# wangyunpeng139/3_ORB_SLAM3_SelfNote

Hardware: AMD Instinct MI355X
Metric: frames/sec ORB extract+match, 752x480 (higher is better)
Workload: dtype u8; 1 GPU; BASELINE configs[2]: extract + SearchByProjection match, 1000x1000 candidates, synthetic frame stream; image=752x480, nfeatures=1000, nlevels=8, batch=256, distinct_frames_per_gpu=2048, streams=4

## Files before the change

### 3_orb_slam3_selfnote_amd/csrc/orb_match_kernels.h

```cpp
#pragma once
#include <hip/hip_runtime.h>
#include <stdint.h>
#include "orb_mfma_util.h"

#define MATCH_NT 256

struct MatchProblemSet {
  const float *kp;
  const uint8_t *desc;
  const float *u_right;
  int frame_stride;
  const int32_t *frame_n; int frame_n_stride; int frame_n_const;
  float min_x, min_y, inv_w, inv_h;
  const uint8_t *qdesc;
  const float *qu, *qv, *qr, *qur;
  const int32_t *qminl, *qmaxl;
  const uint8_t *qflags;
  int query_stride;
  const int32_t *query_n; int query_n_stride; int query_n_const;
  float nnratio; int th_dist; int use_second;
  int32_t *slot; uint8_t *slot_obs; int32_t *match_of_query; int32_t *best_dist; int32_t *nmatches;
  int nleft; const uint8_t *qside; const int32_t *partner; int couple; uint8_t *qany; int serial;
  const int32_t *nleft_dev; int nleft_stride;
  float inv_sigma2[16];
// ... 676 lines not shown
    K l[REFRESH_K];
#pragma unroll
    for (int j = 0; j < REFRESH_K; j++) l[j] = KT::NONE;
    const int minlE = w.checkLevels ? w.minl : -1000, maxlE = w.checkLevels && w.maxl >= 0 ? w.maxl : 1000;
    struct Probe { float x, y, ur; uint32_t bits; int c, pos; };
    auto probe = [&](int pos, bool valid) {
      Probe k;
      k.c = valid ? (int)sPerm[pos] : -1;
      k.pos = valid ? pos : 0;
      const int c = valid ? k.c : 0;
      const bool cl = sOwner[valid ? c : n] == 0u;
      if (LDSCAND) {
        const CandMeta cmeta = cMeta[k.pos];
        k.x = cmeta.x; k.y = cmeta.y; k.ur = cmeta.ur;
        k.bits = cl ? (cmeta.bits & ~(1u << 24)) : cmeta.bits;
      } else {
        k.x = kp[(size_t)c * 7]; k.y = kp[(size_t)c * 7 + 1];
        k.bits = cand_bits(k.x, k.y, __float_as_int(kp[(size_t)c * 7 + 5]), cl, M);
        k.ur = M.u_right ? M.u_right[fo + c] : -1.f;
      }
      return k;
    };
    auto passes = [&](const Probe &k) {
      const int gx = (k.bits >> 8) & 0xff, gy = (k.bits >> 16) & 0xff, oct = k.bits & 0xff;
      int viol = (gx - w.cx0) | (w.cx1 - gx) | (gy - w.cy0) | (w.cy1 - gy) | (oct - minlE) | (maxlE - oct) | k.c;
      viol |= ((k.c >= nleft) == sideR) ? 0 : -1;
      viol |= ~(int)(k.bits << 7);
      const int fpass = __float_as_int(fabsf(k.x - w.u) - w.r) & __float_as_int(fabsf(k.y - w.v) - w.r);
      bool ok = (fpass & ~viol) < 0;
      if (w.stereo) ok = ok && !(k.ur > 0.f && fabsf(w.ur - k.ur) > w.r);
      return ok;
    };
    auto score = [&](const Probe &k) {
      uint32_t d[8];
      if (LDSCAND) {
        const uint4 a = cDesc[2 * k.pos], b = cDesc[2 * k.pos + 1];
        d[0] = a.x; d[1] = a.y; d[2] = a.z; d[3] = a.w; d[4] = b.x; d[5] = b.y; d[6] = b.z; d[7] = b.w;
      } else {
#pragma unroll
        for (int t = 0; t < 8; t++) d[t] = desc[(size_t)k.c * 8 + t];
      }
      int dist = 0;
#pragma unroll
      for (int t = 0; t < 8; t++) dist += __popc(d[t] ^ q8[t]);
      K t = KT::make(dist, cell_of(k.bits), k.c);
      if (t < l[REFRESH_K - 1]) {
#pragma unroll
        for (int j = 0; j < REFRESH_K; j++) {
          const K lo = t < l[j] ? t : l[j];
          const K hi = t < l[j] ? l[j] : t;
          l[j] = lo;
          t = hi;
        }
      }
    };
    const int end = w.live ? sCol[w.cx1 + 1] : 0;
    for (int pos = (w.live ? sCol[w.cx0] : 0) + lane + 128 * part; pos < end; pos += 128 * nparts) {
      const Probe k0 = probe(pos, true);
      const Probe k1 = probe(pos + 64, pos + 64 < end);
      const bool ok0 = passes(k0), ok1 = passes(k1);
      if (ok0) score(k0);
      if (ok1) score(k1);
    }
    K out[REFRESH_K];
#pragma unroll
    for (int j = 0; j < REFRESH_K; j++) {
      out[j] = wave_min_key(l[0]);
      if (l[0] == out[j] && out[j] != KT::NONE) {
#pragma unroll
        for (int t = 0; t + 1 < REFRESH_K; t++) l[t] = l[t + 1];
        l[REFRESH_K - 1] = KT::NONE;
      }
    }
    if (lane == 0) {
#pragma unroll
      for (int j = 0; j < REFRESH_K; j++) sPart[rq][part][j] = out[j];
    }
    (void)target;
  };
  __shared__ int sVoteR;
  constexpr bool WIDE_OK = sizeof(K) == 4;
  constexpr int WN = 64 * NW_;
  constexpr int TKW_WORDS = FUSED && MATCH_TOPK * WN < 3072 ? 3072 : MATCH_TOPK * WN;
  __shared__ __align__(16) K sTkW[WIDE_OK ? TKW_WORDS : 1];
  __shared__ int sRmin[4], sChg[4], sTake, sNm;
  bool wide = false;
  if (FUSED && fusedPair) wide = false;
  else if (WIDE_OK && !M.serial && !M.partner && M.couple == 0 && !M.qside && rforce != SCAN_DENSE) {
    wide = pair_walks<WN>(M, p, n, nq, rforce, &sVoteR);
  }
  if (wide) {
    if (tid == 0) { for (int i = 0; i < 4; i++) { sRmin[i] = 0x7fffffff; sChg[i] = 0; } sTake = 0; sNm = 0; }
    __syncthreads();
    int nmatches = 0;
#ifdef WIDE_STAMPS
    long long ws_build = 0, ws_round = 0, ws_refresh = 0, ws_nround = 0, ws_nrefresh = 0, ws_ncut = 0, ws_t = __builtin_readcyclecounter();
    const long long ws_begin = ws_t;
#define WSTMP(acc) do { const long long t_ = __builtin_readcyclecounter(); acc += t_ - ws_t; ws_t = t_; } while (0)
#else
#define WSTMP(acc) do {} while (0)
#endif
    for (int base = 0; base < nq; base += WN) {
      const int q = base + tid;
      const int cnt = min(WN, nq - base);
      const uint32_t myfl = q < nq ? (M.qflags ? M.qflags[qo + q] : 3u) : 0u;
      const bool ob = (myfl >> 1) & 1u;
      uint32_t qpar[6] = {0, 0, 0, 0, 0, 0}, qd[8] = {0, 0, 0, 0, 0, 0, 0, 0};
#pragma unroll
      for (int j = 0; j < MATCH_TOPK; j++) sTkW[WN * j + tid] = q < nq ? topk[(qo + q) * MATCH_TOPK + j] : KT::NONE;
      if (q < nq) {
        qpar[0] = __float_as_uint(M.qu[qo + q]); qpar[1] = __float_as_uint(M.qv[qo + q]); qpar[2] = __float_as_uint(M.qr[qo + q]);
        qpar[3] = __float_as_uint(M.qur ? M.qur[qo + q] : 0.f);
        qpar[4] = (uint32_t)M.qminl[qo + q]; qpar[5] = (uint32_t)M.qmaxl[qo + q];
        const uint4 *qp = reinterpret_cast<const uint4 *>(M.qdesc + (qo + q) * 32);
        const uint4 a = qp[0], b = qp[1];
        qd[0] = a.x; qd[1] = a.y; qd[2] = a.z; qd[3] = a.w; qd[4] = b.x; qd[5] = b.y; qd[6] = b.z; qd[7] = b.w;
      }
      int eidx[MATCH_TOPK];
      uint32_t vm, oct4;
      int capm1 = MATCH_TOPK - 1, lbDist;
      bool truncated;
      auto load_list = [&]() {
        vm = 0; oct4 = 0;
#pragma unroll
        for (int j = 0; j < MATCH_TOPK; j++) {
          const K t = sTkW[WN * j + tid];
          eidx[j] = n;
          if (t != KT::NONE) {
            const int idx = KT::idx(t);
            eidx[j] = idx;
            vm |= 1u << j;
            oct4 |= (uint32_t)(octave_of(idx) & 0xf) << (4 * j);
          }
        }
        const K last = sTkW[WN * capm1 + tid];
        truncated = last != KT::NONE;
        lbDist = KT::dist(last);
        if (!(myfl & 1u)) { vm = 0; truncated = false; }
      };
      load_list();
      auto refresh = [&](bool want) {
        bool todo = want;
        WSTMP(ws_round);
        for (;;) {
          __syncthreads();
          int slot = -1;
          if (todo) slot = atomicAdd(&sTake, 1);
          const bool take = todo && slot < NW_;
          if (take) {
            uint32_t *R = sReq[slot];
            R[0] = (uint32_t)tid; R[1] = myfl;
#pragma unroll
            for (int t = 0; t < 6; t++) R[2 + t] = qpar[t];
#pragma unroll
            for (int t = 0; t < 8; t++) R[8 + t] = qd[t];
          }
          __syncthreads();
          const int asked = sTake;
          if (asked == 0) break;
          const int m = min(NW_, asked);
          {
            const int np = shares_of(m), mp = NW_ / np, rq = wid & (mp - 1);
            if (rq < m) serve(rq, wid / mp, np);
          }
          __syncthreads();
          if (tid == 0) sTake = 0;
          if (take) {
            static_assert(REFRESH_K == 4, "the merge network below is written for 4 keys");
            auto cx = [](K &lo, K &hi) { const K l = lo < hi ? lo : hi, h = lo < hi ? hi : lo; lo = l; hi = h; };
            const int np = shares_of(m);
            K a[REFRESH_K];
#pragma unroll
            for (int j = 0; j < REFRESH_K; j++) a[j] = sPart[slot][0][j];
            for (int sh = 1; sh < np; sh++) {
#pragma unroll
              for (int j = 0; j < REFRESH_K; j++) {
                const K y = sPart[slot][sh][REFRESH_K - 1 - j];
                a[j] = a[j] < y ? a[j] : y;
              }
              cx(a[0], a[2]); cx(a[1], a[3]);
              cx(a[0], a[1]); cx(a[2], a[3]);
            }
#pragma unroll
            for (int j = 0; j < MATCH_TOPK; j++) sTkW[WN * j + tid] = j < REFRESH_K ? a[j] : KT::NONE;
            todo = false;
            capm1 = REFRESH_K - 1;
            load_list();
          }
#ifdef WIDE_STAMPS
          ws_nrefresh++;
#endif
        }
        WSTMP(ws_refresh);
      };
      uint32_t D = 0;
      int my_bd = 256, res_idx = -1, res_bd = 256;
      int s = 0, par = 0;
      bool first_round = true;
      WSTMP(ws_build);
      while (s < cnt) {
#ifdef WIDE_STAMPS
        ws_ncut++;
#endif
        int r;
        for (;;) {
          const bool pend = tid >= s && tid < cnt;
          const bool post = pend && (D >> 31) && ob;
          const int bidx = (int)(D & 0xfffffu);
          if (post) __hip_atomic_fetch_min(&sOwner[bidx], (uint32_t)(tid + 1), __ATOMIC_RELAXED, __HIP_MEMORY_SCOPE_WORKGROUP);
          __syncthreads();
          uint32_t cm = 0;
#pragma unroll
          for (int j = 0; j < MATCH_TOPK; j++) cm |= (sOwner[eidx[j]] <= (uint32_t)tid ? 1u : 0u) << j;
          const uint32_t mine = sOwner[post ? bidx : n];
          __syncthreads();
          if (post && mine != 0u) sOwner[bidx] = RESOLVE_FREE;
          const uint32_t nD = pend ? decide<KT, WN>(M, sTkW + tid, vm, cm, oct4, truncated, lbDist, &my_bd) : D;
          const bool changed = nD != D;
          D = nD;
          const bool flagged = pend && ((D >> 30) & 1u);
          const int cur = par & 3;
          par++;
#ifdef WIDE_STAMPS
          ws_nround++;
#endif
          if (tid == 0) { sRmin[(cur + 2) & 3] = 0x7fffffff; sChg[(cur + 2) & 3] = 0; }
          if (flagged) atomicMin(&sRmin[cur], tid);
          __syncthreads();
          r = min(sRmin[cur], cnt);
          if (first_round) {
            first_round = false;
            if (r < cnt) {
              refresh(flagged);
              continue;
            }
          }
          if (changed && tid <= r) sChg[cur] = 1;
          __syncthreads();
          if (sChg[cur] == 0) break;
        }
        {
          const bool inpre = tid >= s && tid < r;
          const bool acc = inpre && (D >> 31);
          const int bidx = (int)(D & 0xfffffu);
          nmatches += __popcll(__ballot(acc));
          if (acc) {
            const int32_t sv = (int32_t)(((uint32_t)q << 1) | (ob ? 1u : 0u));
            if (ob) sOwner[bidx] = 0u;
            __hip_atomic_fetch_max(&sSlot[bidx], sv, __ATOMIC_RELAXED, __HIP_MEMORY_SCOPE_WORKGROUP);
          }
          if (inpre) { res_idx = acc ? bidx : -1; res_bd = my_bd <= M.th_dist ? my_bd : 256; }
        }
        s = r;
        if (r < cnt) refresh(tid >= r && tid < cnt && ((D >> 30) & 1u));
        else __syncthreads();
      }
      if (q < nq) {
        if (M.match_of_query) M.match_of_query[qo + q] = res_idx;
        if (M.best_dist) M.best_dist[qo + q] = res_bd;
      }
    }
    WSTMP(ws_round);
#ifdef WIDE_STAMPS
    if (tid == 0 && M.dbg) { long long *d = M.dbg + 16 * (size_t)p; d[0] = ws_build; d[1] = ws_round; d[2] = ws_refresh; d[3] = ws_nround; d[4] = ws_nrefresh; d[5] = ws_ncut; d[6] = ws_t - ws_begin; d[7] = nq; }
#endif
    if (lane == 0 && nmatches) atomicAdd(&sNm, nmatches);
    __syncthreads();
    if (tid == 0 && M.nmatches) M.nmatches[p] = sNm;
    for (int i = tid; i < n; i += 64 * NW_) {
      const int32_t v = sSlot[i];
      if (v >= 0) { slot[i] = v >> 1; slot_obs[i] = (uint8_t)(v & 1); }
    }
    return;
  }
  constexpr int CMP_CAP = 2048 / NW_;
  static_assert(!FUSED || (64 * 8 + 64 * NW_ * REFRESH_K + NW_ * CMP_CAP / 2 + NW_ * MF_TILE) * 4 <= TKW_WORDS * (int)sizeof(K), "work areas exceed the list array");
  uint32_t *sReqD = reinterpret_cast<uint32_t *>(sTkW);
  uint32_t *sPartF = sReqD + 64 * 8;
  uint16_t *sCmpF = reinterpret_cast<uint16_t *>(sPartF + 64 * NW_ * REFRESH_K);
  uint32_t *sSeedF = reinterpret_cast<uint32_t *>(sCmpF + NW_ * CMP_CAP);
  auto serve_mfma = [&](int m) __attribute__((always_inline)) {
    if constexpr (FUSED) {
      const int col = lane & 31, h = lane >> 5;
      const int nin = sCol[64];
      const int lo = (int)(((long long)nin * wid) / NW_), hi = (int)(((long long)nin * (wid + 1)) / NW_);
      uint16_t *cmp = sCmpF + wid * CMP_CAP;
      int kw = 0;
      for (int b0 = lo; b0 < hi; b0 += 64) {
        const int pos = b0 + lane;
        bool keep = false;
        if (pos < hi) keep = !(sRank[pos] & MF_REC_HELD) && sOwner[sPerm[pos]] != 0u;
        const unsigned long long mk = __ballot(keep);
        if (keep) cmp[kw + __popcll(mk & ((1ull << lane) - 1ull))] = (uint16_t)pos;
        kw += __popcll(mk);
      }
      const bool two = m > 32;
      uint32_t q0[4], q1[4];
      {
        const uint4 *r0 = reinterpret_cast<const uint4 *>(sReqD + col * 8), *r1 = reinterpret_cast<const uint4 *>(sReqD + (32 + col) * 8);
        const uint4 a0 = r0[0], b0 = r0[1], a1 = r1[0], b1 = r1[1];
        const uint32_t d0[8] = {a0.x, a0.y, a0.z, a0.w, b0.x, b0.y, b0.z, b0.w}, d1[8] = {a1.x, a1.y, a1.z, a1.w, b1.x, b1.y, b1.z, b1.w};
#pragma unroll
        for (int s = 0; s < 4; s++) {
          q0[s] = ((d0[2 * s] >> (16 * h)) & 0xffffu) | ((d0[2 * s + 1] >> (16 * h)) << 16);
          q1[s] = ((d1[2 * s] >> (16 * h)) & 0xffffu) | ((d1[2 * s + 1] >> (16 * h)) << 16);
        }
      }
      auto bq = [](const uint32_t *q, int s) { return mf_expand16((q[s >> 1] >> (16 * (s & 1))) & 0xffffu, MF_LUT_QUERY); };
      MfList<REFRESH_K> L0, L1;
      L0.init(); L1.init();
      uint32_t *seedw = sSeedF + wid * MF_TILE;
      int npos = 0;
      uint4 na = make_uint4(0u, 0u, 0u, 0u), nb = na;
      if (kw > 0) {
        npos = col < kw ? (int)cmp[col] : 0;
        na = cDesc[2 * npos]; nb = cDesc[2 * npos + 1];
      }
      for (int t0 = 0; t0 < kw; t0 += MF_TILE) {
        const bool have = t0 + col < kw;
#pragma unroll
        for (int s = 0; s < 4; s++) asm("" : "+v"(q0[s]), "+v"(q1[s]));
        const int pos = npos;
        const uint4 da = na, db = nb;
        if (t0 + MF_TILE < kw) {
          const int e2 = t0 + MF_TILE + col;
          npos = e2 < kw ? (int)cmp[e2] : 0;
          na = cDesc[2 * npos]; nb = cDesc[2 * npos + 1];
        }
        if (h == 0) seedw[col] = have ? sRank[pos] : MF_REC_UNUSABLE;
        const uint32_t dd[8] = {da.x, da.y, da.z, da.w, db.x, db.y, db.z, db.w};
        mf_v4i A[8];
#pragma unroll
        for (int s = 0; s < 8; s++) A[s] = mf_expand16((dd[s] >> (16 * h)) & 0xffffu, MF_LUT_CAND);
        mf_v16i c;
#pragma unroll
        for (int g = 0; g < 4; g++) {
          const mf_v4i v4 = *reinterpret_cast<const mf_v4i *>(&seedw[8 * g + 4 * h]);
          c[4 * g] = v4[0]; c[4 * g + 1] = v4[1]; c[4 * g + 2] = v4[2]; c[4 * g + 3] = v4[3];
        }
        mf_v16i acc0 = c;
#pragma unroll
        for (int s = 0; s < 8; s++) acc0 = __builtin_amdgcn_mfma_i32_32x32x32_i8(A[s], bq(q0, s), acc0, 0, 0, 0);
        L0.take(acc0);
        if (two) {
          mf_v16i acc1 = c;
#pragma unroll
          for (int s = 0; s < 8; s++) acc1 = __builtin_amdgcn_mfma_i32_32x32x32_i8(A[s], bq(q1, s), acc1, 0, 0, 0);
          L1.take(acc1);
        }
      }
      static_assert(REFRESH_K == 4, "the merge network below is written for 4 keys");
      uint32_t mg[REFRESH_K];
#pragma unroll
      for (int j = 0; j < REFRESH_K; j++) {
        const uint32_t send = h ? L0.top[REFRESH_K - 1 - j] : L1.top[REFRESH_K - 1 - j];
        const uint32_t other = (uint32_t)__shfl_xor((int)send, 32, 64);
        mg[j] = min(h ? L1.top[j] : L0.top[j], other);
      }
      auto cxu = [](uint32_t &a, uint32_t &b) { const uint32_t l = min(a, b), g2 = max(a, b); a = l; b = g2; };
      cxu(mg[0], mg[2]); cxu(mg[1], mg[3]);
      cxu(mg[0], mg[1]); cxu(mg[2], mg[3]);
      const int req = h * 32 + col;
      if (req < m) *reinterpret_cast<uint4 *>(sPartF + ((size_t)req * NW_ + wid) * REFRESH_K) = make_uint4(mg[0], mg[1], mg[2], mg[3]);
    }
  };
  auto fold_mfma = [&](int rank, K *colp ) {
    if constexpr (FUSED) {
      auto cxu = [](uint32_t &a, uint32_t &b) { const uint32_t l = min(a, b), g2 = max(a, b); a = l; b = g2; };
      const uint4 *sh = reinterpret_cast<const uint4 *>(sPartF + (size_t)rank * NW_ * REFRESH_K);
      uint4 v = sh[0];
      uint32_t a[REFRESH_K] = {v.x, v.y, v.z, v.w};
#pragma unroll
      for (int w2 = 1; w2 < NW_; w2++) {
        v = sh[w2];
        a[0] = min(a[0], v.w); a[1] = min(a[1], v.z); a[2] = min(a[2], v.y); a[3] = min(a[3], v.x);
        cxu(a[0], a[2]); cxu(a[1], a[3]);
        cxu(a[0], a[1]); cxu(a[2], a[3]);
      }
#pragma unroll
      for (int j = 0; j < MATCH_TOPK; j++) {
        K o = KT::NONE;
        if (j < REFRESH_K && a[j] < MF_KEY_LIMIT) o = (K)(((a[j] >> 11) << 23) | (uint32_t)sPerm[a[j] & 0x7ffu]);
        colp[64 * j] = o;
      }
    }
  };
#ifdef RESOLVE_STAMPS
  long long t_round = 0, t_refresh = 0, n_refresh = 0, n_batch = 0, t_chunk = 0, n_round = 0, t_sub[6] = {0, 0, 0, 0, 0, 0}, sub_m = 0;
  long long t0 = __builtin_readcyclecounter();
#endif
  if (wid != 0) {
    for (;;) {
      __syncthreads();
      const int m = sCmd;
      if (m < 0) break;
      if (FUSED && fusedPair) serve_mfma(m);
      else {
        const int np = shares_of(m), mp = NW_ / np, rq = wid & (mp - 1);
        if (rq < m) serve(rq, wid / mp, np);
      }
      __syncthreads();
    }
  } else {
    int nmatches = 0;
    for (int base = 0; base < nq; base += 64) {
#ifdef RESOLVE_STAMPS
      long long tc0 = __builtin_readcyclecounter();
#endif
      const int q = base + lane;
      const int cnt = min(64, nq - base);
      uint32_t myfl = q < nq ? (M.qflags ? M.qflags[qo + q] : 3u) : 0u;
      if (M.qside && q < nq && M.qside[qo + q]) myfl |= 0x100u;
      if (M.couple == 2 && (q & 1) && q < nq && !M.qany[qo + q - 1]) myfl &= ~1u;
      const bool ob = (myfl >> 1) & 1u;
      uint32_t qpar[6] = {0, 0, 0, 0, 0, 0}, qd[8] = {0, 0, 0, 0, 0, 0, 0, 0};
#pragma unroll
      for (int j = 0; j < MATCH_TOPK; j++) sTk[64 * j + lane] = (q < nq && !(FUSED && fusedPair)) ? topk[(qo + q) * MATCH_TOPK + j] : KT::NONE;
      if (q < nq) {
        qpar[0] = __float_as_uint(M.qu[qo + q]); qpar[1] = __float_as_uint(M.qv[qo + q]); qpar[2] = __float_as_uint(M.qr[qo + q]);
        qpar[3] = __float_as_uint(M.qur ? M.qur[qo + q] : 0.f);
        qpar[4] = (uint32_t)M.qminl[qo + q]; qpar[5] = (uint32_t)M.qmaxl[qo + q];
        const uint4 *qp = reinterpret_cast<const uint4 *>(M.qdesc + (qo + q) * 32);
        const uint4 a = qp[0], b = qp[1];
        qd[0] = a.x; qd[1] = a.y; qd[2] = a.z; qd[3] = a.w; qd[4] = b.x; qd[5] = b.y; qd[6] = b.z; qd[7] = b.w;
        if (FUSED && fusedPair && !load_query(M, qo, q).live) myfl &= ~1u;
      }
      int eidx[MATCH_TOPK];
      uint32_t vm, oct4;
      int capm1 = MATCH_TOPK - 1, lbDist;
      bool truncated;
      auto load_list = [&]() {
        vm = 0; oct4 = 0;
#pragma unroll
        for (int j = 0; j < MATCH_TOPK; j++) {
          const K t = sTk[64 * j + lane];
          eidx[j] = n;
          if (t != KT::NONE) {
            const int idx = KT::idx(t);
            eidx[j] = idx;
            vm |= 1u << j;
            oct4 |= (uint32_t)(octave_of(idx) & 0xf) << (4 * j);
          }
        }
        const K last = sTk[64 * capm1 + lane];
        truncated = last != KT::NONE;
        lbDist = KT::dist(last);
        if (!(myfl & 1u)) { vm = 0; truncated = false; }
      };
      load_list();
      auto refresh = [&](unsigned long long F) {
#ifdef RESOLVE_STAMPS
        long long ts0 = __builtin_readcyclecounter(), ts1 = ts0;
#endif
        const bool mineF = (F >> lane) & 1ull;
        unsigned long long todo = F;
        if (FUSED && fusedPair && todo) {
          const int rank = __popcll(todo & ((1ull << lane) - 1ull));
          if (mineF) {
            uint4 *R = reinterpret_cast<uint4 *>(sReqD + rank * 8);
            R[0] = make_uint4(qd[0], qd[1], qd[2], qd[3]);
            R[1] = make_uint4(qd[4], qd[5], qd[6], qd[7]);
          }
          const int m = (int)__popcll(todo);
          if (lane == 0) sCmd = m;
          __syncthreads();
          serve_mfma(m);
          __syncthreads();
          if (mineF) fold_mfma(rank, sTk + lane);
          todo = 0ull;
#ifdef RESOLVE_STAMPS
          n_batch++;
#endif
        }
        while (todo) {
          const int rank = __popcll(todo & ((1ull << lane) - 1ull));
          const bool take = ((todo >> lane) & 1ull) && rank < NW_;
          if (take) {
            uint32_t *R = sReq[rank];
            R[0] = (uint32_t)lane; R[1] = myfl;
#pragma unroll
            for (int t = 0; t < 6; t++) R[2 + t] = qpar[t];
#pragma unroll
            for (int t = 0; t < 8; t++) R[8 + t] = qd[t];
          }
          const int m = min(NW_, (int)__popcll(todo));
          if (lane == 0) sCmd = m;
#ifdef RESOLVE_STAMPS
          long long tq = __builtin_readcyclecounter(); t_sub[0] += tq - ts1; ts1 = tq; sub_m += m;
#endif
          __syncthreads();
#ifdef RESOLVE_STAMPS
          tq = __builtin_readcyclecounter(); t_sub[1] += tq - ts1; ts1 = tq;
#endif
          const int np = shares_of(m);
          serve(0, 0, np);
#ifdef RESOLVE_STAMPS
          tq = __builtin_readcyclecounter(); t_sub[2] += tq - ts1; ts1 = tq;
#endif
          __syncthreads();
#ifdef RESOLVE_STAMPS
          tq = __builtin_readcyclecounter(); t_sub[3] += tq - ts1; ts1 = tq;
#endif
          if (take) {
            static_assert(REFRESH_K == 4, "the merge network below is written for 4 keys");
            auto cx = [](K &lo, K &hi) { const K l = lo < hi ? lo : hi, h = lo < hi ? hi : lo; lo = l; hi = h; };
            K a[REFRESH_K];
#pragma unroll
            for (int j = 0; j < REFRESH_K; j++) a[j] = sPart[rank][0][j];
            for (int sh = 1; sh < np; sh++) {
#pragma unroll
              for (int j = 0; j < REFRESH_K; j++) {
                const K y = sPart[rank][sh][REFRESH_K - 1 - j];
                a[j] = a[j] < y ? a[j] : y;
              }
              cx(a[0], a[2]); cx(a[1], a[3]);
              cx(a[0], a[1]); cx(a[2], a[3]);
            }
#pragma unroll
            for (int j = 0; j < MATCH_TOPK; j++) sTk[64 * j + lane] = j < REFRESH_K ? a[j] : KT::NONE;
          }
          todo &= ~__ballot(take);
#ifdef RESOLVE_STAMPS
          n_batch++;
          tq = __builtin_readcyclecounter(); t_sub[4] += tq - ts1; ts1 = tq;
#endif
        }
        if (mineF) capm1 = REFRESH_K - 1;
        load_list();
#ifdef RESOLVE_STAMPS
        t_sub[5] += __builtin_readcyclecounter() - ts1;
        t_refresh += __builtin_readcyclecounter() - ts0; n_refresh += __popcll(F);
#endif
      };
      if (FUSED && fusedPair) {
        const unsigned long long want = __ballot(q < nq && (myfl & 1u));
        if (want) refresh(want);
      }
      uint32_t D = 0;
      int my_bd = 256, res_idx = -1, res_bd = 256;
#ifdef RESOLVE_STAMPS
      t_chunk += __builtin_readcyclecounter() - tc0;
#endif
      int s = 0;
      bool first_round = !M.serial;
      while (s < cnt) {
#ifdef RESOLVE_STAMPS
        long long tr0 = __builtin_readcyclecounter();
#endif
        const int hi = M.serial ? s + 1 : cnt;
        if (M.serial) refresh(1ull << s);
        int r;
        unsigned long long flagged;
        for (;;) {
          const bool pend = lane >= s && lane < hi;
          const bool post = pend && (D >> 31) && ob;
          const int bidx = (int)(D & 0xfffffu);
          int pidx = n;
          if (M.partner && post) { const int pr = sPartner[bidx]; pidx = pr == 0xffff ? n : pr; }
          if (post) __hip_atomic_fetch_min(&sOwner[bidx], (uint32_t)(lane + 1), __ATOMIC_RELAXED, __HIP_MEMORY_SCOPE_WORKGROUP);
          if (M.partner && pidx != n) __hip_atomic_fetch_min(&sOwner[pidx], (uint32_t)(lane + 1), __ATOMIC_RELAXED, __HIP_MEMORY_SCOPE_WORKGROUP);
          __builtin_amdgcn_wave_barrier();
          uint32_t cm = 0;
#pragma unroll
          for (int j = 0; j < MATCH_TOPK; j++) cm |= (sOwner[eidx[j]] <= (uint32_t)lane ? 1u : 0u) << j;
          const uint32_t mine = sOwner[post ? bidx : n];
          uint32_t mineP = 0u;
          if (M.partner) mineP = sOwner[pidx];
          __builtin_amdgcn_wave_barrier();
          if (post && mine != 0u) sOwner[bidx] = RESOLVE_FREE;
          if (M.partner && pidx != n && mineP != 0u) sOwner[pidx] = RESOLVE_FREE;
          __builtin_amdgcn_wave_barrier();
          uint32_t nD = pend ? decide<KT>(M, sTk + lane, vm, cm, oct4, truncated, lbDist, &my_bd) : D;
          if (M.couple == 1) {
            const uint32_t leftD = (uint32_t)__builtin_amdgcn_update_dpp(0, (int)D, 0x111, 0xf, 0xf, true);
            if (pend && (lane & 1) && ((leftD >> 29) & 1u)) { nD = 0; my_bd = 256; }
          }
          const bool changed = nD != D;
          D = nD;
          flagged = __ballot(pend && ((D >> 30) & 1u));
#ifdef RESOLVE_STAMPS
          n_round++;
#endif
          if (first_round) {
            first_round = false;
            if (flagged) {
#ifdef RESOLVE_STAMPS
              t_round += __builtin_readcyclecounter() - tr0;
#endif
              refresh(flagged);
#ifdef RESOLVE_STAMPS
              tr0 = __builtin_readcyclecounter();
#endif
              continue;
            }
          }
          r = flagged ? (int)__builtin_ctzll(flagged) : hi;
          if (!__ballot(changed && lane <= r)) break;
        }
        {
          const bool inpre = lane >= s && lane < r;
          const bool acc = inpre && (D >> 31);
          const int bidx = (int)(D & 0xfffffu);
          nmatches += __popcll(__ballot(acc));
          if (acc) {
            const int32_t sv = (int32_t)(((uint32_t)q << 1) | (ob ? 1u : 0u));
            if (ob) sOwner[bidx] = 0u;
            __hip_atomic_fetch_max(&sSlot[bidx], sv, __ATOMIC_RELAXED, __HIP_MEMORY_SCOPE_WORKGROUP);
            if (M.partner) {
              const int pr = sPartner[bidx];
              if (pr != 0xffff) {
                sOwner[pr] = ob ? 0u : RESOLVE_FREE;
                __hip_atomic_fetch_max(&sSlot[pr], sv, __ATOMIC_RELAXED, __HIP_MEMORY_SCOPE_WORKGROUP);
              }
            }
          }
          if (M.partner) nmatches += __popcll(__ballot(acc && sPartner[acc ? bidx : 0] != 0xffff));
          if (inpre) { res_idx = acc ? bidx : -1; res_bd = my_bd <= M.th_dist ? my_bd : 256; }
        }
        __builtin_amdgcn_wave_barrier();
#ifdef RESOLVE_STAMPS
        t_round += __builtin_readcyclecounter() - tr0;
#endif
        s = r;
        if (r < hi) refresh(flagged);
      }
      if (q < nq) {
        if (M.match_of_query) M.match_of_query[qo + q] = res_idx;
        if (M.best_dist) M.best_dist[qo + q] = res_bd;
      }
    }
#ifdef RESOLVE_STAMPS
    if (lane == 0 && M.dbg) { long long *d = M.dbg + 16 * (size_t)p; d[0] = n_batch; d[1] = t_chunk; d[2] = t_round; d[3] = t_refresh; d[4] = n_refresh; d[5] = __builtin_readcyclecounter() - t0; d[6] = nq; d[7] = n_round; for (int i = 0; i < 6; i++) d[8 + i] = t_sub[i]; d[14] = sub_m; }
#endif
    if (lane == 0) { sCmd = -1; if (M.nmatches) M.nmatches[p] = nmatches; }
    __syncthreads();
  }
  __syncthreads();
  for (int i = tid; i < n; i += 64 * NW_) {
    const int32_t v = sSlot[i];
    if (v >= 0) { slot[i] = v >> 1; slot_obs[i] = (uint8_t)(v & 1); }
  }
}

template <typename KT>
__global__ __launch_bounds__(64) void k_init_resolve(MatchProblemSet M, const typename KT::T *topk, int th_low) {
  typedef typename KT::T K;
  extern __shared__ __align__(16) uint32_t smem_init[];
  __shared__ K sTk[MATCH_TOPK * 64];
  const int lane = threadIdx.x;
  const int p = blockIdx.x;
  const int n = M.frame_n ? M.frame_n[(size_t)p * M.frame_n_stride] : M.frame_n_const;
  const int nq = M.query_n ? M.query_n[(size_t)p * M.query_n_stride] : M.query_n_const;
  const size_t fo = (size_t)p * M.frame_stride, qo = (size_t)p * M.query_stride;
  const float *kp = M.kp + fo * 7;
  const uint32_t *desc = reinterpret_cast<const uint32_t *>(M.desc + fo * 32);
  uint16_t *sVMD = reinterpret_cast<uint16_t *>(smem_init);
  for (int i = lane; i < n; i += 64) sVMD[i] = 0xffff;
  __builtin_amdgcn_s_barrier();
  int nacc = 0;
  for (int base = 0; base < nq; base += 64) {
    const int q = base + lane, cnt = min(64, nq - base);
#pragma unroll
    for (int j = 0; j < MATCH_TOPK; j++) sTk[64 * j + lane] = q < nq ? topk[(qo + q) * MATCH_TOPK + j] : KT::NONE;
    int res_idx = -1, res_bd = 256;
    for (int i = 0; i < cnt; i++) {
      const K k = lane < MATCH_TOPK ? sTk[64 * lane + i] : KT::NONE;
      const bool valid = k != KT::NONE;
      const int c = valid ? KT::idx(k) : 0, d = KT::dist(k);
      const bool vis = valid && (int)sVMD[c] > d;
      const uint32_t b = (uint32_t)__ballot(vis) & ((1u << MATCH_TOPK) - 1u);
      const int found = __popc(b);
      const int j1 = b ? __builtin_ctz(b) : 0, j2 = (b & (b - 1u)) ? __builtin_ctz(b & (b - 1u)) : 0;
      int bd = found > 0 ? __builtin_amdgcn_readlane(d, j1) : 0x7fffffff;
      int bd2 = found > 1 ? __builtin_amdgcn_readlane(d, j2) : 0x7fffffff;
      int best = found > 0 ? __builtin_amdgcn_readlane(c, j1) : -1;
      const K last = KT::readlane(k, MATCH_TOPK - 1);
      const bool truncated = last != KT::NONE;
      const int lbDist = KT::dist(last);
      bool rescan = false;
      if (truncated) {
        if (found == 0) rescan = lbDist <= th_low;
        else if (found == 1) rescan = bd <= th_low && !((float)bd < (float)lbDist * M.nnratio);
      }
      if (rescan) {
        const QueryWin w = load_query(M, qo, base + i);
// ... 323 lines not shown
```

### 3_orb_slam3_selfnote_amd/csrc/orb_mfma_util.h

```cpp
#pragma once
#include <hip/hip_runtime.h>
#include <stdint.h>

typedef int mf_v4i __attribute__((ext_vector_type(4)));
typedef int mf_v16i __attribute__((ext_vector_type(16)));

#define MF_NT 256
#define MF_TILE 32
#define MF_REC_BASE (1u << 18)
#define MF_REC_HELD (1u << 30)
#define MF_REC_UNUSABLE ((1u << 18) + MF_REC_HELD)
#define MF_KEY_LIMIT (1u << 20)

__device__ __forceinline__ uint32_t mf_med3(uint32_t a, uint32_t b, uint32_t c) { return max(min(a, b), min(max(a, b), c)); }

__device__ __forceinline__ mf_v4i mf_expand16(uint32_t hw, uint32_t lut) {
  mf_v4i o;
#pragma unroll
  for (int i = 0; i < 4; i++) {
    const uint32_t nib = (hw >> (4 * i)) & 0xfu;
    const uint32_t t = (nib * 0x00204081u) & 0x01010101u;
    o[i] = (int)__builtin_amdgcn_perm(0u, lut, t);
  }
  return o;
}
#define MF_LUT_CAND 0x0000E020u
#define MF_LUT_QUERY 0x000020E0u

template <int K>
struct MfList {
  uint32_t top[K];
  __device__ __forceinline__ void init() {
#pragma unroll
    for (int j = 0; j < K; j++) top[j] = 0xffffffffu;
  }
  __device__ __forceinline__ void insert(uint32_t t) {
#pragma unroll
    for (int j = K - 1; j >= 1; j--) top[j] = mf_med3(top[j - 1], top[j], t);
    top[0] = min(top[0], t);
  }
  __device__ __forceinline__ void take(const mf_v16i &k) {
#pragma unroll
    for (int r = 0; r < 16; r++) insert((uint32_t)k[r]);
  }
};
```

Baseline: 282,100 frames/s.

## Compute Hamming distances with FP4 scaled MFMA instead of int8 MFMA

Replaces the int8 32x32x32 MFMA Hamming-distance computation in the fused refresh path with the MI355X scaled f8f6f4 MFMA in FP4 mode. Each descriptor bit is expanded to a signed FP4 nibble, which halves the number of MFMA issues per tile (4 instead of 8) and removes the 16-bit LUT expansion work. Accumulation switches to float, and keys are recovered from the float bit patterns through a new take overload and mf4_key conversion. Correctness depends on the scale encoding and on the float ordering matching the previous integer key ordering, which is subtle.

```diff
diff --git a/3_orb_slam3_selfnote_amd/csrc/orb_match_kernels.h b/3_orb_slam3_selfnote_amd/csrc/orb_match_kernels.h
--- a/3_orb_slam3_selfnote_amd/csrc/orb_match_kernels.h
+++ b/3_orb_slam3_selfnote_amd/csrc/orb_match_kernels.h
@@ -1002,14 +1002,13 @@
         const uint32_t d0[8] = {a0.x, a0.y, a0.z, a0.w, b0.x, b0.y, b0.z, b0.w}, d1[8] = {a1.x, a1.y, a1.z, a1.w, b1.x, b1.y, b1.z, b1.w};
 #pragma unroll
         for (int s = 0; s < 4; s++) {
-          q0[s] = ((d0[2 * s] >> (16 * h)) & 0xffffu) | ((d0[2 * s + 1] >> (16 * h)) << 16);
-          q1[s] = ((d1[2 * s] >> (16 * h)) & 0xffffu) | ((d1[2 * s + 1] >> (16 * h)) << 16);
-        }
-      }
-      auto bq = [](const uint32_t *q, int s) { return mf_expand16((q[s >> 1] >> (16 * (s & 1))) & 0xffffu, MF_LUT_QUERY); };
+          q0[s] = ~(h ? d0[2 * s + 1] : d0[2 * s]);
+          q1[s] = ~(h ? d1[2 * s + 1] : d1[2 * s]);
+        }
+      }
       MfList<REFRESH_K> L0, L1;
       L0.init(); L1.init();
-      uint32_t *seedw = sSeedF + wid * MF_TILE;
+      float *seedw = reinterpret_cast<float *>(sSeedF + wid * MF_TILE);
       int npos = 0;
       uint4 na = make_uint4(0u, 0u, 0u, 0u), nb = na;
       if (kw > 0) {
@@ -1027,25 +1026,25 @@
           npos = e2 < kw ? (int)cmp[e2] : 0;
           na = cDesc[2 * npos]; nb = cDesc[2 * npos + 1];
         }
-        if (h == 0) seedw[col] = have ? sRank[pos] : MF_REC_UNUSABLE;
+        if (h == 0) seedw[col] = mf4_seed(have ? sRank[pos] : MF_REC_UNUSABLE);
         const uint32_t dd[8] = {da.x, da.y, da.z, da.w, db.x, db.y, db.z, db.w};
-        mf_v4i A[8];
-#pragma unroll
-        for (int s = 0; s < 8; s++) A[s] = mf_expand16((dd[s] >> (16 * h)) & 0xffffu, MF_LUT_CAND);
-        mf_v16i c;
+        mf_v4i A[4];
+#pragma unroll
+        for (int s = 0; s < 4; s++) A[s] = mf4_expand32(h ? dd[2 * s + 1] : dd[2 * s]);
+        mf_v16f c;
 #pragma unroll
         for (int g = 0; g < 4; g++) {
-          const mf_v4i v4 = *reinterpret_cast<const mf_v4i *>(&seedw[8 * g + 4 * h]);
-          c[4 * g] = v4[0]; c[4 * g + 1] = v4[1]; c[4 * g + 2] = v4[2]; c[4 * g + 3] = v4[3];
-        }
-        mf_v16i acc0 = c;
-#pragma unroll
-        for (int s = 0; s < 8; s++) acc0 = __builtin_amdgcn_mfma_i32_32x32x32_i8(A[s], bq(q0, s), acc0, 0, 0, 0);
+          const float4 v4 = *reinterpret_cast<const float4 *>(&seedw[8 * g + 4 * h]);
+          c[4 * g] = v4.x; c[4 * g + 1] = v4.y; c[4 * g + 2] = v4.z; c[4 * g + 3] = v4.w;
+        }
+        mf_v16f acc0 = c;
+#pragma unroll
+        for (int s = 0; s < 4; s++) acc0 = mf4_mfma(A[s], mf4_expand32(q0[s]), acc0);
         L0.take(acc0);
         if (two) {
-          mf_v16i acc1 = c;
-#pragma unroll
-          for (int s = 0; s < 8; s++) acc1 = __builtin_amdgcn_mfma_i32_32x32x32_i8(A[s], bq(q1, s), acc1, 0, 0, 0);
+          mf_v16f acc1 = c;
+#pragma unroll
+          for (int s = 0; s < 4; s++) acc1 = mf4_mfma(A[s], mf4_expand32(q1[s]), acc1);
           L1.take(acc1);
         }
       }
@@ -1080,7 +1079,8 @@
 #pragma unroll
       for (int j = 0; j < MATCH_TOPK; j++) {
         K o = KT::NONE;
-        if (j < REFRESH_K && a[j] < MF_KEY_LIMIT) o = (K)(((a[j] >> 11) << 23) | (uint32_t)sPerm[a[j] & 0x7ffu]);
+        const uint32_t key = j < REFRESH_K ? mf4_key(a[j]) : 0xffffffffu;
+        if (key < MF_KEY_LIMIT) o = (K)(((key >> 11) << 23) | (uint32_t)sPerm[key & 0x7ffu]);
         colp[64 * j] = o;
       }
     }
diff --git a/3_orb_slam3_selfnote_amd/csrc/orb_mfma_util.h b/3_orb_slam3_selfnote_amd/csrc/orb_mfma_util.h
--- a/3_orb_slam3_selfnote_amd/csrc/orb_mfma_util.h
+++ b/3_orb_slam3_selfnote_amd/csrc/orb_mfma_util.h
@@ -27,6 +27,26 @@
 #define MF_LUT_CAND 0x0000E020u
 #define MF_LUT_QUERY 0x000020E0u
 
+typedef int mf_v8i __attribute__((ext_vector_type(8)));
+typedef float mf_v16f __attribute__((ext_vector_type(16)));
+#define MF4_SIGN 0x88888888u
+#define MF4_MAG 0x44444444u
+#define MF4_SCALE 0x83838383
+#define MF4_KEY_LIMIT_BITS 0x49800000u
+
+__device__ __forceinline__ mf_v4i mf4_expand32(uint32_t w) {
+  mf_v4i o;
+#pragma unroll
+  for (int j = 0; j < 4; j++) o[j] = (int)(((w << (3 - j)) | MF4_MAG) & (MF4_SIGN | MF4_MAG));
+  return o;
+}
+__device__ __forceinline__ mf_v16f mf4_mfma(const mf_v4i &a, const mf_v4i &b, const mf_v16f &c) {
+  const mf_v8i a8 = {a[0], a[1], a[2], a[3], 0, 0, 0, 0}, b8 = {b[0], b[1], b[2], b[3], 0, 0, 0, 0};
+  return __builtin_amdgcn_mfma_scale_f32_32x32x64_f8f6f4(a8, b8, c, 4 , 4 , 0, MF4_SCALE, 0, MF4_SCALE);
+}
+__device__ __forceinline__ float mf4_seed(uint32_t rec) { return (float)rec; }
+__device__ __forceinline__ uint32_t mf4_key(uint32_t bits) { return bits < MF4_KEY_LIMIT_BITS ? (uint32_t)__uint_as_float(bits) : 0xffffffffu; }
+
 template <int K>
 struct MfList {
   uint32_t top[K];
@@ -43,4 +63,8 @@
 #pragma unroll
     for (int r = 0; r < 16; r++) insert((uint32_t)k[r]);
   }
+  __device__ __forceinline__ void take(const mf_v16f &k) {
+#pragma unroll
+    for (int r = 0; r < 16; r++) insert(__float_as_uint(k[r]));
+  }
 };
```

Result: faster. 294,300 frames/s, median of 6 (+4.3%).
